# lyeemax/IS-VINS

Measured on AMD Instinct MI355X. Metric: sliding-window solves/sec (11 KF, ~300 landmarks), higher is better.
Workload: dtype f64; 1 GPU; 1024 independent synthetic sliding windows per GPU (N=11 KF, Nvo=5, L=300 landmarks, F~1070 reprojection factors each; BASELINE config 4 batch of config-2 windows), full backendOptimization(): NUM_ITERATIONS=10 dogleg iterations + update() + double2vector + MargForward/MargBackward on every window; windows_per_gpu=1024, windows_total=1024, frames=11, landmarks=300, factors_total=1095427

## Files before the change

is-vins_amd/backend.py:

```python
import ctypes as C
import os
import subprocess

import numpy as np

from . import abi

CSRC = os.path.join(os.path.dirname(os.path.abspath(__file__)), "csrc")
LIB_PATH = os.environ.get("ISVINS_LIB") or os.path.join(CSRC, "libisvins_hip.so")
_lib = None

STATUS = {0: "ISV_OK", -1: "ISV_ERR_INVALID_ARG", -2: "ISV_ERR_CAPACITY", -3: "ISV_ERR_NONFINITE",
          -4: "ISV_ERR_DEVICE", -5: "ISV_ERR_UNSUPPORTED"}
EXPORTS = ["isv_abi_version", "isv_backend_create", "isv_backend_destroy", "isv_backend_last_error",
           "isv_backend_optimize", "isv_backend_optimize_batch", "isv_backend_init_factor_graph", "isv_backend_init_factor_graph_batch", "isv_backend_triangulate", "isv_backend_solve_odometry_batch", "isv_backend_linearize",
           "isv_batch_upload", "isv_batch_optimize", "isv_batch_linearize", "isv_batch_download",
           "isv_batch_sync", "isv_batch_last_timing", "isv_batch_last_counts",
           "isv_result_record_doubles", "isv_batch_pack_results",
           "isv_backend_seq_enable", "isv_backend_seq_seed", "isv_backend_seq_frame", "isv_backend_seq_download", "isv_backend_seq_flush", "isv_backend_seq_marg"]


class BackendError(RuntimeError):
    pass


def build(force=False):
    import fcntl
    if not force and subprocess.call(["make", "-s", "-q", "-C", CSRC]) == 0:
        return LIB_PATH
    with open(os.path.join(CSRC, ".build.lock"), "w") as lock:
        fcntl.flock(lock, fcntl.LOCK_EX)
        try:
            if force:
                subprocess.check_call(["make", "-s", "-C", CSRC, "clean"])
            subprocess.check_call(["make", "-s", "-C", CSRC])
        finally:
            fcntl.flock(lock, fcntl.LOCK_UN)
    return LIB_PATH


def load_library():
    global _lib
    if _lib is not None:
        return _lib
    if not os.path.exists(LIB_PATH):
        raise BackendError(f"HIP extension missing: {LIB_PATH} (run __graft_entry__.build())")
    try:
        import torch
    except Exception:
        pass
    lib = C.CDLL(LIB_PATH)
    vp = C.c_void_p
    wpp = C.POINTER(C.POINTER(abi.isv_window_t))
    dp = abi.c_double_p
    lib.isv_abi_version.restype = C.c_int
    lib.isv_backend_create.argtypes = [C.POINTER(abi.isv_config_t), C.POINTER(vp)]
    lib.isv_backend_destroy.argtypes = [vp]; lib.isv_backend_destroy.restype = None
    lib.isv_backend_last_error.argtypes = [vp]; lib.isv_backend_last_error.restype = C.c_char_p
    lib.isv_backend_optimize.argtypes = [vp, C.POINTER(abi.isv_window_t), C.POINTER(abi.isv_summary_t), C.POINTER(abi.isv_marg_result_t)]
    lib.isv_backend_optimize_batch.argtypes = [vp, C.c_int32, wpp, C.POINTER(abi.isv_summary_t), C.POINTER(abi.isv_marg_result_t)]
    lib.isv_backend_init_factor_graph.argtypes = [vp, C.POINTER(abi.isv_window_t), C.POINTER(abi.isv_summary_t), dp]
    lib.isv_backend_init_factor_graph_batch.argtypes = [vp, C.c_int32, wpp, C.POINTER(abi.isv_summary_t), dp]
    lib.isv_backend_triangulate.argtypes = [vp, C.c_int32, wpp]
    lib.isv_backend_solve_odometry_batch.argtypes = [vp, C.c_int32, wpp, C.POINTER(abi.isv_summary_t), C.POINTER(abi.isv_marg_result_t)]
    lib.isv_backend_linearize.argtypes = [vp, C.POINTER(abi.isv_window_t), dp, dp, dp]
    lib.isv_batch_upload.argtypes = [vp, C.c_int32, wpp]
    lib.isv_batch_optimize.argtypes = [vp, C.c_int32]
    lib.isv_batch_linearize.argtypes = [vp, C.c_int32]
    lib.isv_batch_download.argtypes = [vp, C.c_int32, wpp, C.POINTER(abi.isv_summary_t), C.POINTER(abi.isv_marg_result_t)]
    lib.isv_batch_sync.argtypes = [vp]
    lib.isv_batch_last_timing.argtypes = [vp, dp]
    lib.isv_batch_last_counts.argtypes = [vp, C.POINTER(C.c_int64)]
    lib.isv_debug_read.argtypes = [vp, C.c_int32, dp, C.c_int64]
    lib.isv_result_record_doubles.argtypes = [vp]; lib.isv_result_record_doubles.restype = C.c_int64
    lib.isv_batch_pack_results.argtypes = [vp, vp, vp]
    _lib = lib
    return lib


class Backend:
    def __init__(self, n_frames=11, n_vo=5, max_landmarks=1000, max_obs=None, max_batch=1, **kw):
        self.lib = load_library()
        self.cfg = abi.make_config(n_frames, n_vo, max_landmarks=max_landmarks, max_obs=max_obs, max_batch=max_batch, **kw)
        self.h = C.c_void_p()
        rc = self.lib.isv_backend_create(C.byref(self.cfg), C.byref(self.h))
        if rc != 0:
            raise BackendError(f"isv_backend_create failed: {STATUS.get(rc, rc)} (a MI355X and the HIP extension are required; there is no CPU path)")
        self._keep = None

    def close(self):
        if self.h:
            self.lib.isv_backend_destroy(self.h)
            self.h = C.c_void_p()

    def __del__(self):
        try:
            self.close()
        except Exception:
            pass

    def _check(self, rc, what):
        if rc != 0:
            msg = self.lib.isv_backend_last_error(self.h)
            raise BackendError(f"{what}: {STATUS.get(rc, rc)} {msg.decode() if msg else ''}")

    def _ptrs(self, windows):
        cs = [w.c() for w in windows]
        arr = (C.POINTER(abi.isv_window_t) * len(cs))(*[C.pointer(c) for c in cs])
        self._keep = (cs, arr, windows)
        return arr

    def optimize(self, window):
        s, m = self.optimize_batch([window])
        return s[0], m[0]

    def optimize_batch(self, windows):
        n = len(windows)
        sums = (abi.isv_summary_t * n)(); margs = (abi.isv_marg_result_t * n)()
        self._check(self.lib.isv_backend_optimize_batch(self.h, n, self._ptrs(windows), sums, margs), "optimize_batch")
        return list(sums), list(margs)

    def linearize(self, window):
        F, N = window.n_factors, window.N
        ps = np.zeros((max(F, 1), abi.ISV_PROJ_STRIP)); im = np.zeros((N - 1, abi.ISV_IMU_STRIP)); cost = np.zeros(1)
        cw = window.c()
        self._check(self.lib.isv_backend_linearize(self.h, C.byref(cw), abi._p(ps), abi._p(im), abi._p(cost)), "linearize")
# ... 15 lines not shown
        n = len(windows)
        sums = (abi.isv_summary_t * n)(); kld = np.zeros(n)
        self._check(self.lib.isv_backend_init_factor_graph_batch(self.h, n, self._ptrs(windows), sums, abi._p(kld)), "init_factor_graph_batch")
        for w in windows:
            w.n_rollpitch = 0; w.margin_old = 0
        return list(sums), kld

    def triangulate(self, windows):
        self._check(self.lib.isv_backend_triangulate(self.h, len(windows), self._ptrs(windows)), "triangulate")

    def marshal(self, windows):
        return self._ptrs(windows)

    def upload(self, windows, ptrs=None):
        self._check(self.lib.isv_batch_upload(self.h, len(windows), ptrs if ptrs is not None else self._ptrs(windows)), "upload")
        self._n = len(windows)

    def run_optimize(self, sync=True, profile=False):
        self._check(self.lib.isv_batch_optimize(self.h, (1 if sync else 0) | (2 if profile else 0)), "batch_optimize")

    def run_linearize(self, sync=True):
        self._check(self.lib.isv_batch_linearize(self.h, 1 if sync else 0), "batch_linearize")

    def sync(self):
        self._check(self.lib.isv_batch_sync(self.h), "sync")

    def download(self, windows, ptrs=None, as_list=True):
        n = len(windows)
        sums = (abi.isv_summary_t * n)(); margs = (abi.isv_marg_result_t * n)()
        self._check(self.lib.isv_batch_download(self.h, n, ptrs if ptrs is not None else self._ptrs(windows), sums, margs), "download")
        return (list(sums), list(margs)) if as_list else (sums, margs)

    def record_doubles(self):
        return int(self.lib.isv_result_record_doubles(self.h))

    def pack_results(self, device_ptr, stream=None):
        s = C.c_void_p(-1) if stream is None else C.c_void_p(int(stream))
        self._check(self.lib.isv_batch_pack_results(self.h, C.c_void_p(device_ptr), s), "pack_results")

    def last_timing(self):
        out = np.zeros(8)
        self._check(self.lib.isv_batch_last_timing(self.h, abi._p(out)), "last_timing")
        return out

    def last_counts(self):
        out = (C.c_int64 * 8)()
        self._check(self.lib.isv_batch_last_counts(self.h, out), "last_counts")
        return list(out)

    def debug_read(self, what, count):
        out = np.zeros(count)
        self._check(self.lib.isv_debug_read(self.h, what, abi._p(out), count), "debug_read")
        return out
```

is-vins_amd/csrc/isv_backend.hip:

```cpp
#include <hip/hip_runtime.h>
#include <atomic>
#include <chrono>
#include <cstdio>
#include <cstdlib>
#include <cstring>
#include <string>
#include <thread>
#include <sched.h>
#include <vector>
#include <algorithm>
#include "isv_device_types.h"
#include "isv_kernels.h"

#include "isv_batch_buffers.h"

extern "C" int isv_abi_version(void) { return ISV_ABI_VERSION; }

extern "C" const char *isv_backend_last_error(const isv_backend_t *h) { return h ? h->err.c_str() : "null handle"; }

extern "C" void isv_backend_destroy(isv_backend_t *h) {
    if (!h) return;
    (void)hipSetDevice(h->device);
    if (h->graph_exec) (void)hipGraphExecDestroy(h->graph_exec);
    if (h->seq && h->seq_free) h->seq_free(h->seq);
// ... 759 lines not shown
        double *q = o + 16 * N + maxL;
        q[0] = st.x_cost; q[1] = st.initial_cost; q[2] = st.iteration; q[3] = st.termination; q[4] = st.num_successful;
        q[5] = st.radius; q[6] = d.header0[w]; q[7] = Lw;
    }
}

extern "C" int64_t isv_result_record_doubles(const isv_backend_t *h) {
    return h ? 16 * (int64_t)h->cfg.n_frames + h->cfg.max_landmarks + 8 : 0;
}

extern "C" int isv_batch_pack_results(isv_backend_t *h, void *device_dst, void *stream) {
    if (!h || !device_dst || !h->resident) return ISV_ERR_INVALID_ARG;
    ENTER(h);
    DevBatch &d = h->d;
    hipStream_t dst_stream = stream == ISV_STREAM_OF_HANDLE ? h->stream : (hipStream_t)stream;
    if (dst_stream != h->stream) {
        HIPCHK(h, hipEventRecord(h->pk[0], h->stream));
        HIPCHK(h, hipStreamWaitEvent(dst_stream, h->pk[0], 0));
    }
    hipLaunchKernelGGL(k_pack_results, dim3(d.B), dim3(256), 0, dst_stream, d, (double *)device_dst, isv_result_record_doubles(h), h->cfg.max_landmarks);
    HIPCHK(h, hipGetLastError());
    if (dst_stream != h->stream) {
        HIPCHK(h, hipEventRecord(h->pk[1], dst_stream));
        HIPCHK(h, hipStreamWaitEvent(h->stream, h->pk[1], 0));
    }
    return ISV_OK;
}

extern "C" int isv_debug_read(isv_backend_t *h, int32_t what, double *out, int64_t count) {
    if (!h || !out) return ISV_ERR_INVALID_ARG;
    ENTER(h);
    DevBatch &d = h->d; hipStream_t st = h->stream;
    const double *src = nullptr;
    const size_t B = h->capB, NI = B * (size_t)(d.N - 1);
    size_t cap = 0;
    switch (what) {
    case 0: src = d.prior_strip; cap = B * (size_t)d.prior_strip_sz; break;
    case 1: src = d.prior_cost; cap = B * (size_t)d.n_prior_slots; break;
    case 2: src = d.imu_sqrt; cap = NI * 225; break;
    case 3: src = d.fcost; cap = h->capF; break;
    case 4: src = d.imu_cost; cap = NI; break;
    case 5: src = d.pose; cap = B * (size_t)d.N * 7; break;
    case 6: src = d.lam; cap = h->capL; break;
    case 7: src = d.cost; cap = B; break;
    case 22: src = d.strip_ex; cap = h->capF * 12; if (!src) return ISV_ERR_INVALID_ARG; break;
    default: return isv_solver_debug_read(h->d, st, what, out, count, h->capB, h->capL, h->err);
    }
    if (count < 0 || (size_t)count > cap) { h->err = "isv_debug_read: count exceeds the buffer"; return ISV_ERR_INVALID_ARG; }
    if (count == 0) return ISV_OK;
    D2H(out, src, count);
    HIPCHK(h, hipStreamSynchronize(st));
    return ISV_OK;
}
```

is-vins_amd/csrc/isv_kernels.h:

```cpp
#pragma once
#include <hip/hip_runtime.h>
#include <string>
#include <vector>
#include "isv_device_types.h"
#include "isv_solve_plan.h"

__global__ void k_vector2double(DevBatch d);
__global__ void k_imu_prep(DevBatch d, const int32_t *sel);
template <int MODE> __global__ void k_proj_linearize(DevBatch d, const double *pose_src, const double *lam_src, double *fcost_out, int gate);
template <bool JAC> __global__ void k_imu_linearize(DevBatch d, const double *pose_src, const double *sb_src, double *cost_out, int gate);
template <bool JAC> __global__ void k_prior_linearize(DevBatch d, const double *pose_src, const double *sb_src, double *cost_out, int gate);
__global__ void k_cost_reduce(DevBatch d, const double *fcost, const double *imu_cost, const double *prior_cost, double *out, int gate);

struct SolverHost {
    SolveEnv env;
    SolveDevice dev;
    HandlePlan plan;
    UploadShape upload;
    const void *fn[KR_COUNT] = {};
};
const void *isv_solver_kernel(SolverRole r, KernelInst i, bool ex, int nt);
UploadPlan isv_solver_plan_upload(SolverHost &hc, const UploadShape &u);
int isv_solver_alloc(DevBatch &d, SolverHost &hc, size_t B, size_t L, size_t F, std::vector<void *> &allocs, std::string &err);
int isv_solver_enqueue(DevBatch &d, const SolverHost &hc, hipStream_t st, hipStream_t st2, hipEvent_t *fj, int64_t *counts, hipEvent_t *prof_ev, std::string &err);
__global__ void k_triangulate(DevBatch d);
template <bool EX, int LGW> __global__ void k_lin_gram(DevBatch d);
template <int NT, int TPW> __global__ void k_schur_split(DevBatch d, int Gs, int GrMax);
template <int NT, int TPW> __global__ void k_rank1_split(DevBatch d, int GrMax);
__global__ void k_schur_fold(DevBatch d, int GrMax, int NT, int from_partials);
__global__ void k_imu_raw(DevBatch d, const double *pose_src, const double *sb_src, int gate);
__global__ void k_imu_weight(DevBatch d, double *cost_out, int gate);
#define ISV_PROF_FAMILIES 6
enum { ISV_CNT_LINEARIZE, ISV_CNT_SOLVE, ISV_CNT_ELIM, ISV_CNT_WINDOW_ITERS, ISV_CNT_FUSED_VISUAL, ISV_CNT_FUSED_CONTROL, ISV_CNT_SOLVE_ST, ISV_CNT_SPLIT_GROUPS };
struct SolverStage { SolveState *st; double *tc, *tr, *ts; int32_t *ta; isv_marg_result_t *marg; };
hipError_t isv_raise_dynamic_lds(const void *fn, int device, size_t lds);
int isv_upload_build_enqueue(DevBatch &d, const int32_t *optr, const double *obs_raw, int lcap, hipStream_t st);
int isv_solver_download(struct isv_backend *h, int n, isv_summary_t *summary, isv_marg_result_t *marg);
void isv_solver_unpack_window(const SolverStage &stage, int b, isv_summary_t *summary, isv_marg_result_t *marg);
int isv_solver_debug_read(DevBatch &d, hipStream_t st, int what, double *out, int64_t count, size_t capB, size_t capL, std::string &err);
```

is-vins_amd/csrc/isv_marg.hip:

```cpp
#include <hip/hip_runtime.h>
#include "isv_kernels.h"
#include "isv_device_math.h"
#include "isv_proj_factor.h"
#include "isv_prior_factor.h"

#define MT 64
#ifdef ISV_STAMP
#define MSTAMP(k) do { if (t == 0) { unsigned long long now_ = wall_clock64(); d.dbg[(size_t)w * 64 + 32 + (k)] += (double)(now_ - t_last); t_last = now_; } } while (0)
#else
#define MSTAMP(k) do {} while (0)
#endif
#define SYNC() __syncthreads()
template <bool WV> DEV void tsync() {
    if constexpr (WV) {
        __builtin_amdgcn_fence(__ATOMIC_RELEASE, "workgroup");
        __builtin_amdgcn_wave_barrier();
        __builtin_amdgcn_fence(__ATOMIC_ACQUIRE, "workgroup");
    } else __syncthreads();
}

DEV double jr_rsqrt(double x) { double r = __builtin_amdgcn_rsq(x); const double h = 0.5 * x; r = r * fma(-(h * r), r, 1.5); r = r * fma(-(h * r), r, 1.5); return r; }
DEV double jr_rcp(double x) { double r = __builtin_amdgcn_rcp(x); r = r * fma(-x, r, 2.0); r = r * fma(-x, r, 2.0); return r; }
DEV void jr_params(double app, double aqq, double apq, bool rot, double &c, double &sn) {
    const double theta = ((aqq - app) * 0.5) * jr_rcp(apq);
    const double th2 = fma(theta, theta, 1.0);
    const double tv = (theta >= 0 ? 1.0 : -1.0) * jr_rcp(fma(th2, jr_rsqrt(th2), fabs(theta)));
    const double cc = jr_rsqrt(fma(tv, tv, 1.0));
    c = rot ? cc : 1.0; sn = rot ? tv * cc : 0.0;
}
DEV void jr_block(double ca, double sa, double cb, double sb, double b00, double b01, double b10, double b11,
                  double &o00, double &o01, double &o10, double &o11) {
    const double c00 = fma(cb, b00, -(sb * b01)), c01 = fma(sb, b00, cb * b01);
    const double c10 = fma(cb, b10, -(sb * b11)), c11 = fma(sb, b10, cb * b11);
    o00 = fma(ca, c00, -(sa * c10)); o01 = fma(ca, c01, -(sa * c11));
    o10 = fma(sa, c00, ca * c10); o11 = fma(sa, c01, ca * c11);
}
DEV void jr_vec(double c, double sn, double vp, double vq, double &op, double &oq) { op = fma(c, vp, -(sn * vq)); oq = fma(sn, vp, c * vq); }

template <int TS = MT, bool WV = false>
DEV void w_mm(const double *A, const double *B, double *C, int m, int k, int n, int t) {
    for (int e = t; e < m * n; e += TS) { const int i = e / n, j = e % n; double s = 0; for (int p = 0; p < k; p++) s += A[i * k + p] * B[p * n + j]; C[e] = s; }
    tsync<WV>();
}
template <int TS = MT, bool WV = false>
DEV void w_mm_tn(const double *A, const double *B, double *C, int m, int k, int n, int t) {
    for (int e = t; e < m * n; e += TS) { const int i = e / n, j = e % n; double s = 0; for (int p = 0; p < k; p++) s += A[p * m + i] * B[p * n + j]; C[e] = s; }
    tsync<WV>();
}
template <int TS = MT, bool WV = false>
DEV void w_mm_nt(const double *A, const double *B, double *C, int m, int k, int n, int t) {
    for (int e = t; e < m * n; e += TS) { const int i = e / n, j = e % n; double s = 0; for (int p = 0; p < k; p++) s += A[i * k + p] * B[j * k + p]; C[e] = s; }
    tsync<WV>();
}
template <int TS = MT, bool WV = false>
DEV void w_inv(const double *A, int n, double *Inv, double *W, int *piv, int t) {
    const int n2 = 2 * n;
    for (int e = t; e < n * n2; e += TS) { const int i = e / n2, j = e % n2; W[e] = (j < n) ? A[i * n + j] : ((j - n) == i ? 1.0 : 0.0); }
// ... 408 lines not shown
        SYNC();
        int rank = 6;
        if (t == 0) {
            double Aq[36]; for (int k = 0; k < 36; k++) Aq[k] = Lp[k];
            double pv[6], maxp = 0; rank = 0;
            for (int k = 0; k < 6; k++) pv[k] = 0;
            for (int k = 0; k < 6; k++) {
                int pi = k, pj = k; double best = 0;
                for (int i = k; i < 6; i++) for (int j = k; j < 6; j++) if (fabs(Aq[i * 6 + j]) > best) { best = fabs(Aq[i * 6 + j]); pi = i; pj = j; }
                pv[k] = best; if (best > maxp) maxp = best;
                if (best == 0) break;
                for (int j = 0; j < 6; j++) { const double tmp2 = Aq[k * 6 + j]; Aq[k * 6 + j] = Aq[pi * 6 + j]; Aq[pi * 6 + j] = tmp2; }
                for (int i = 0; i < 6; i++) { const double tmp2 = Aq[i * 6 + k]; Aq[i * 6 + k] = Aq[i * 6 + pj]; Aq[i * 6 + pj] = tmp2; }
                for (int i = k + 1; i < 6; i++) { const double f = Aq[i * 6 + k] / Aq[k * 6 + k]; for (int j = k; j < 6; j++) Aq[i * 6 + j] -= f * Aq[k * 6 + j]; }
            }
            for (int k = 0; k < 6; k++) if (pv[k] > 1e-16 * maxp) rank++;
            piv[1] = rank;
        }
        SYNC();
        rank = piv[1];
        if (rank == 6) {
            w_inv(Lp, 6, cov, Wk + 600, piv, t);
            w_mm(sJ, cov, T, 6, 6, 6, t);
            w_mm_nt(T, sJ, covi, 6, 6, 6, t);
        } else {
            for (int e = t; e < 36; e += MT) JU[e] = Lp[e];
            SYNC();
            w_jacobi(JU, 6, wv, Vv, nullptr, t);
            if (t < 6) keep[t] = wv[t] > d.alpha_cut;
            SYNC();
            w_project_cov(sJ, 6, 6, Vv, wv, keep, JU, covi, t);
        }
        w_inv(covi, 6, X, Wk + 600, piv, t);
        double kld = 0;
        if (rank == 6) {
            double *phi = Wk + 448, *pc = Wk + 512;
            w_mm_tn(sJ, X, T, 6, 6, 6, t);
            w_mm(T, sJ, phi, 6, 6, 6, t);
            w_mm(phi, cov, pc, 6, 6, 6, t);
            const double dphi = w_det(phi, 6, Wk + 900, piv, t), dcov = w_det(cov, 6, Wk + 900, piv, t);
            double a = 0; for (int k = 0; k < 6; k++) a += pc[k * 6 + k];
            kld = 0.5 * (a - log(dphi) - log(dcov) - 6);
        }
        w_chol_upper(X, 6, JU, Wk + 800, t);
        for (int e = t; e < 36; e += MT) fp.sqrt_info[e] = JU[e];
        if (t == 0) { out.forward_kld = kld; out.n_marg_landmarks = n0; out.valid = 1; }
        SYNC();
    }
    MSTAMP(4);
}
template __global__ void k_marg_fwd<64>(DevBatch);
template __global__ void k_marg_fwd<256>(DevBatch);

template <int NC>
DEV void jacobi4(double *sA, double *sV, int t) {
    constexpr int n = NC, m = n + (n & 1), half = m / 2, NI = half * half, NN = n * n;
    static_assert(NI <= 128 && half <= 32, "one item per lane of two wavefronts");
    __shared__ double red[8], sink[2], rc[2][32], rs[2][32];
    __shared__ int rp[2][32], rq[2][32];
    for (int e = t; e < NN; e += 256) sV[e] = (e / n == e % n) ? 1.0 : 0.0;
    __syncthreads();
    const bool is_block = t < 128;
    const int e = is_block ? t : t - 128;
    const bool valid = e < NI;
    const int i0 = valid ? e / half : 0, i1 = valid ? e % half : 0;
    auto params = [&](int r, int buf) {
        if (t < half) {
            const int k = t;
            int a = r + k, b = r + m - 1 - k;
            a = a >= m - 1 ? a - (m - 1) : a;
            b = b >= m - 1 ? b - (m - 1) : b;
            a = k == 0 ? m - 1 : a; b = k == 0 ? r : b;
            const int p = a < b ? a : b, q0 = a < b ? b : a, q = q0 < n ? q0 : p;
            const double apq = sA[p * n + q], aqq = sA[q * n + q], app = sA[p * n + p];
            double c, sn;
            jr_params(app, aqq, apq, p != q && apq != 0.0, c, sn);
            rp[buf][k] = p; rq[buf][k] = q; rc[buf][k] = c; rs[buf][k] = sn;
        }
    };
    bool polish = false;
    for (int sweep = 0; sweep < 30; sweep++) {
        double off = 0, dg = 0;
        for (int x = t; x < NN; x += 256) { const int i = x / n, j = x % n; const double v = sA[x]; if (j > i) off += v * v; else if (i == j) dg += v * v; }
        for (int o = 32; o > 0; o >>= 1) { off += __shfl_xor(off, o); dg += __shfl_xor(dg, o); }
        if ((t & 63) == 0) { red[(t >> 6) * 2] = off; red[(t >> 6) * 2 + 1] = dg; }
        params(0, 0);
        __syncthreads();
        off = red[0] + red[2] + red[4] + red[6]; dg = red[1] + red[3] + red[5] + red[7];
        if (off <= 1e-60 || off <= 1e-32 * dg || polish) break;
        if (off <= 1e-28 * dg) polish = true;
        for (int r = 0; r < m - 1; r++) {
            const int buf = r & 1;
            if (is_block) {
                const int p1 = rp[buf][i0], q1 = rq[buf][i0], p2 = rp[buf][i1], q2 = rq[buf][i1];
                const double ca = rc[buf][i0], sa = rs[buf][i0], cb = rc[buf][i1], sb = rs[buf][i1];
                double *const a00 = valid ? sA + p1 * n + p2 : sink, *const a01 = valid ? sA + p1 * n + q2 : sink;
                double *const a10 = valid ? sA + q1 * n + p2 : sink, *const a11 = valid ? sA + q1 * n + q2 : sink;
                const double b00 = *a00, b01 = *a01, b10 = *a10, b11 = *a11;
                double o00, o01, o10, o11;
                jr_block(ca, sa, cb, sb, b00, b01, b10, b11, o00, o01, o10, o11);
                *a00 = o00; *a01 = o01; *a10 = o10; *a11 = o11;
            } else {
                const int p = rp[buf][i0], q = rq[buf][i0];
                const double c = rc[buf][i0], sn = rs[buf][i0];
                const int k0 = 2 * i1, k1 = (2 * i1 + 1 < n) ? 2 * i1 + 1 : k0;
                double *const v0p = valid ? sV + k0 * n + p : sink + 1, *const v0q = valid ? sV + k0 * n + q : sink + 1;
                double *const v1p = valid ? sV + k1 * n + p : sink + 1, *const v1q = valid ? sV + k1 * n + q : sink + 1;
                const double a0 = *v0p, b0 = *v0q, a1 = *v1p, b1 = *v1q;
                double r0p, r0q, r1p, r1q;
                jr_vec(c, sn, a0, b0, r0p, r0q); jr_vec(c, sn, a1, b1, r1p, r1q);
                *v0p = r0p; *v0q = r0q; *v1p = r1p; *v1q = r1q;
            }
            __syncthreads();
            if (r + 1 < m - 1) { params(r + 1, buf ^ 1); __syncthreads(); }
        }
    }
}
template <int NC>
__global__ __launch_bounds__(256) void k_marg_jacobi(DevBatch d) {
    constexpr int n = NC, NN = n * n;
    __shared__ double sA[NN + 1], sV[NN + 1];
    const int w = blockIdx.x, t = threadIdx.x;
    if (!d.margin_old[w] || ISV_SEQ_IDLE(d, w)) return;
#ifdef ISV_STAMP
    unsigned long long t_last = wall_clock64();
#endif
    double *const ws = d.marg_ws + (size_t)w * ISV_MARG_WS;
    for (int e = t; e < NN; e += 256) sA[e] = ws[e];
    jacobi4<NC>(sA, sV, t);
    for (int x = t; x < NN; x += 256) ws[896 + x] = sV[x];
    if (t < n) ws[1344 + t] = sA[t * n + t];
#ifdef ISV_STAMP
    if (t == 0) d.dbg[(size_t)w * 64 + 32 + 6] += (double)(wall_clock64() - t_last);
#endif
}
template __global__ void k_marg_jacobi<21>(DevBatch);

enum { IRJ_RIT = 1, IRJ_S = 2, IRJ_B1 = 4, IRJ_T = 8, IRJ_B2 = 16, IRJ_ALL = 31 };
DEV void imu_raw_jac(const DevBatch &d, size_t f, const double *pi, const double *si, double *M1, int pieces) {
    const double *rec = d.imu_in + f * ISV_IMU_IN;
    const double *pj = pi + 7, *sj = si + 9;
    Quat Qi = q_from_pose(pi), Qj = q_from_pose(pj), Qii = q_inv(Qi);
    const double dt = rec[IMU_DT];
    double dbg[3], tt[3], u[3], o1[3], o2[3], RiT[9], S1[9], S2[9], B1[9], B2[9], L[9], Rr[9], T[9];
    Quat dq = Quat{rec[IMU_DQ + 3], rec[IMU_DQ], rec[IMU_DQ + 1], rec[IMU_DQ + 2]};
    Quat cdq = dq;
    if (pieces & (IRJ_B1 | IRJ_B2)) {
        for (int k = 0; k < 3; k++) dbg[k] = si[6 + k] - rec[IMU_LBG + k];
        m3v(rec + IMU_DQ_DBG, dbg, tt);
        cdq = q_mul(dq, q_delta(tt));
    }
    if (pieces & IRJ_RIT) q_to_R(Qii, RiT);
    if (pieces & IRJ_S) {
        for (int k = 0; k < 3; k++) u[k] = 0.5 * d.G[k] * dt * dt + pj[k] - pi[k] - si[k] * dt;
        q_rot(Qii, u, o1);
        for (int k = 0; k < 3; k++) u[k] = d.G[k] * dt + sj[k] - si[k];
        q_rot(Qii, u, o2);
        skew3(o1, S1); skew3(o2, S2);
    }
    if (pieces & IRJ_B1) {
        Quat aq = q_mul(q_inv(Qj), Qi);
        qleft33(aq, L); qright33(cdq, Rr); m3_mul(L, Rr, B1);
        const double av[3] = {aq.x, aq.y, aq.z}, bv[3] = {cdq.x, cdq.y, cdq.z};
        for (int r = 0; r < 3; r++) for (int c = 0; c < 3; c++) B1[r * 3 + c] += av[r] * (-bv[c]);
    }
    if (pieces & IRJ_T) {
        qleft33(q_mul(q_mul(q_inv(Qj), Qi), dq), L);
        m3_mul(L, rec + IMU_DQ_DBG, T);
    }
    if (pieces & IRJ_B2) qleft33(q_mul(q_mul(q_inv(cdq), Qii), Qj), B2);
    for (int a = 0; a < 3; a++) for (int b = 0; b < 3; b++) {
        const int ab = a * 3 + b;
        if (pieces & IRJ_RIT) {
            M1[(0 + a) * 30 + 0 + b] = -RiT[ab]; M1[(0 + a) * 30 + 6 + b] = -RiT[ab] * dt; M1[(6 + a) * 30 + 6 + b] = -RiT[ab];
            M1[(0 + a) * 30 + 15 + b] = RiT[ab]; M1[(6 + a) * 30 + 21 + b] = RiT[ab];
        }
        if (pieces & IRJ_S) { M1[(0 + a) * 30 + 3 + b] = S1[ab]; M1[(6 + a) * 30 + 3 + b] = S2[ab]; }
        if (pieces & IRJ_B1) M1[(3 + a) * 30 + 3 + b] = -B1[ab];
        if (pieces & IRJ_T) M1[(3 + a) * 30 + 12 + b] = -T[ab];
        if (pieces & IRJ_B2) M1[(3 + a) * 30 + 18 + b] = B2[ab];
    }
}
DEV void imu_raw_copies(const DevBatch &d, size_t f, double *M1, int ab) {
    const double *rec = d.imu_in + f * ISV_IMU_IN;
    const int a = ab / 3, b = ab % 3;
    M1[(0 + a) * 30 + 9 + b] = -rec[IMU_DP_DBA + ab]; M1[(0 + a) * 30 + 12 + b] = -rec[IMU_DP_DBG + ab];
    M1[(6 + a) * 30 + 9 + b] = -rec[IMU_DV_DBA + ab]; M1[(6 + a) * 30 + 12 + b] = -rec[IMU_DV_DBG + ab];
    M1[(9 + a) * 30 + 9 + b] = (a == b) ? -1.0 : 0.0; M1[(12 + a) * 30 + 12 + b] = (a == b) ? -1.0 : 0.0;
    M1[(9 + a) * 30 + 24 + b] = (a == b) ? 1.0 : 0.0; M1[(12 + a) * 30 + 27 + b] = (a == b) ? 1.0 : 0.0;
// ... 74 lines not shown
    } else if (t == 0) {
        const size_t f = (size_t)w * (N - 1) + (v - 1);
        imu_raw_jac(d, f, pose + 7 * (v - 1), sb + 9 * (v - 1), M1, IRJ_ALL);
        for (int ab = 0; ab < 9; ab++) imu_raw_copies(d, f, M1, ab);
    }
    SYNC();
    {
        const double *S = d.imu_sqrt + ((size_t)w * (N - 1) + (v - 1)) * 225;
        for (int e = t; e < 450; e += NTH) { const int a = e / 30, c = e % 30; double s = 0; for (int k = 0; k < 15; k++) s += S[a * 15 + k] * M1[k * 30 + c]; M2[e] = s; }
        SYNC();
        for (int e = t; e < 900; e += NTH) {
            const int a = e / 30, b = e % 30;
            const int ga = (a < 15) ? 15 + a : a - 15, gb = (b < 15) ? 15 + b : b - 15;
            double s = 0; for (int k = 0; k < 15; k++) s += M2[k * 30 + a] * M2[k * 30 + b];
            Lam[ga * 30 + gb] += s;
        }
        SYNC();
    }
    double *Lp = M1;
    {
        double *A99 = Wk, *Ainv = Wk + 100;
        for (int e = t; e < 81; e += NTH) A99[e] = Lam[(21 + e / 9) * 30 + 21 + e % 9];
        SYNC();
        if constexpr (PART == 3) { if (wid == 0) w_inv<64, true>(A99, 9, Ainv, Wk + 200, piv, lane); SYNC(); }
        else w_inv(A99, 9, Ainv, Wk + 200, piv, t);
        for (int e = t; e < 441; e += NTH) {
            const int a = e / 21, b = e % 21; double s = Lam[a * 30 + b];
#pragma unroll SCHUR_UNROLL
            for (int p = 0; p < 9; p++) { double tt = 0; for (int q = 0; q < 9; q++) tt += Ainv[p * 9 + q] * Lam[b * 30 + 21 + q]; s -= Lam[a * 30 + 21 + p] * tt; }
            Lp[e] = s;
        }
        SYNC();
    }
    if constexpr (PART == 3) {
        for (int e = t; e < 441; e += NTH) Jr[e] = recovered_jac_entry(e / 21, e % 21, sJ, wv);
    } else {
        for (int e = t; e < 441; e += MT) Jr[e] = 0.0;
        SYNC();
        if (t == 0) {
            double BmBy[9];
            recovered_jac(pose, sb, v, rp, vb, gp, sJ, BmBy);
            for (int a = 0; a < 6; a++) for (int b = 0; b < 6; b++) { Jr[a * 21 + 15 + b] += sJ[a * 6 + b]; Jr[a * 21 + b] += sJ[36 + a * 6 + b]; }
            for (int a = 0; a < 9; a++) Jr[(6 + a) * 21 + 6 + a] += 1.0;
            for (int a = 0; a < 2; a++) for (int b = 0; b < 3; b++) Jr[(15 + a) * 21 + 18 + b] += BmBy[a * 3 + b];
            for (int a = 0; a < 3; a++) Jr[(17 + a) * 21 + 15 + a] += 1.0;
            for (int b = 0; b < 3; b++) Jr[20 * 21 + 18 + b] += BmBy[6 + b];
        }
    }
    SYNC();
    if constexpr (PART == 0) for (int e = t; e < 441; e += MT) { ws[e] = Lp[e]; ws[448 + e] = Jr[e]; }
    MSTAMP(5);
    if constexpr (PART == 3) {
        for (int e = t; e < 441; e += NTH) M2[e] = Lp[e];
        jacobi4<21>(M2, Vv, t);
        if (t < 21) { const double ev = M2[t * 21 + t]; wv[t] = ev; keep[t] = ev > d.alpha_cut; }
        SYNC();
        MSTAMP(6);
    }
    if constexpr (PART == 2) {
        for (int e = t; e < 441; e += MT) M2[e] = Lp[e];
        SYNC();
        w_jacobi(M2, 21, wv, Vv, nullptr, t);
        if (t < 21) keep[t] = wv[t] > d.alpha_cut;
        SYNC();
        MSTAMP(6);
    }
    }
    if constexpr (PART == 1) {
        for (int e = t; e < 441; e += MT) { Jr[e] = ws[448 + e]; Vv[e] = ws[896 + e]; }
        if (t < 21) { const double ev = ws[1344 + t]; wv[t] = ev; keep[t] = ev > d.alpha_cut; }
        SYNC();
    }
    if constexpr (PART != 0) {
    {
        double *Sg = Wk, *Xi = Wk + 100, *Xall = M1;
        for (int e = t; e < 441; e += NTH) Xall[e] = 0.0;
        SYNC();
#define RECOVER_ON(WV, TT, R0, NR, DST, JUp, Sgp, Xip, Wp, Lp_, PV)                                                     \
        do {                                                                                                            \
            w_project_cov<MT, WV>(Jr + (R0) * 21, (NR), 21, Vv, wv, keep, (JUp), (Sgp), (TT));                          \
            w_inv<MT, WV>((Sgp), (NR), (Xip), (Wp), (PV), (TT));                                                        \
            for (int e = (TT); e < (NR) * (NR); e += MT) Xall[((R0) + e / (NR)) * 21 + (R0) + e % (NR)] = (Xip)[e];    \
            tsync<WV>();                                                                                                \
            if ((DST) != nullptr) {                                                                                     \
                w_chol_upper<MT, WV>((Xip), (NR), (Sgp), (Lp_), (TT));                                                  \
                for (int e = (TT); e < (NR) * (NR); e += MT) (DST)[e] = (Sgp)[e];                                       \
                tsync<WV>();                                                                                            \
            }                                                                                                           \
        } while (0)
#define RECOVER(R0, NR, DST) RECOVER_ON(false, t, R0, NR, DST, JU, Sg, Xi, Wk + 300, Wk + 200, piv)
        double *const no_dst = nullptr;
        if constexpr (PART == 3) {
            if (wid == 0) RECOVER_ON(true, lane, 6, 9, vb.sqrt_info, JU + 6 * 21, Sg, Xi, Wk + 300, Wk + 200, piv);
            else if (wid == 1) RECOVER_ON(true, lane, 0, 6, rp.sqrt_info, JU, M2, M2 + 36, M2 + 72, M2 + 144, piv + 1);
            else if (wid == 2) {
                RECOVER_ON(true, lane, 15, 2, gp.sqrt_info, JU + 15 * 21, M2 + 200, M2 + 210, M2 + 220, M2 + 240, piv + 2);
                RECOVER_ON(true, lane, 17, 3, no_dst, JU + 17 * 21, M2 + 200, M2 + 210, M2 + 220, M2 + 240, piv + 2);
                RECOVER_ON(true, lane, 20, 1, no_dst, JU + 20 * 21, M2 + 200, M2 + 210, M2 + 220, M2 + 240, piv + 2);
            }
            SYNC();
        } else {
            RECOVER(0, 6, rp.sqrt_info);
            RECOVER(6, 9, vb.sqrt_info);
            RECOVER(15, 2, gp.sqrt_info);
            RECOVER(17, 3, no_dst);
            RECOVER(20, 1, no_dst);
        }
// ... 201 lines not shown
```

Baseline: 211,600 windows/s.

## Pipeline Jacobi rotation parameters with double-buffered matrix to halve barriers per round

Restructures the 4-wavefront parallel Jacobi eigensolver used in marginalization. One wavefront now computes the next round's rotation parameters speculatively, gathering 2x2 blocks via DPP quad broadcasts from precomputed offset tables, while the others apply the current rotations into a ping-pong buffer. This removes the second barrier per round and the serialized params step. Eigenvector updates are regrouped so that lanes own rows. It adds a second 21x21 shared buffer, heavier index math, and a debug hook for testing the kernel in isolation.

```diff
diff --git a/is-vins_amd/backend.py b/is-vins_amd/backend.py
--- a/is-vins_amd/backend.py
+++ b/is-vins_amd/backend.py
@@ -72,6 +72,8 @@
     lib.isv_batch_last_timing.argtypes = [vp, dp]
     lib.isv_batch_last_counts.argtypes = [vp, C.POINTER(C.c_int64)]
     lib.isv_debug_read.argtypes = [vp, C.c_int32, dp, C.c_int64]
+    if hasattr(lib, "isv_debug_jacobi"):
+        lib.isv_debug_jacobi.argtypes = [vp, C.c_int32, dp, C.c_int64, dp, dp]
     lib.isv_result_record_doubles.argtypes = [vp]; lib.isv_result_record_doubles.restype = C.c_int64
     lib.isv_batch_pack_results.argtypes = [vp, vp, vp]
     _lib = lib
@@ -193,3 +195,9 @@
         out = np.zeros(count)
         self._check(self.lib.isv_debug_read(self.h, what, abi._p(out), count), "debug_read")
         return out
+
+    def debug_jacobi(self, mats, waves=4):
+        a = np.ascontiguousarray(mats, dtype=np.float64).reshape(-1, 21, 21)
+        V = np.zeros_like(a); w = np.zeros((a.shape[0], 21))
+        self._check(self.lib.isv_debug_jacobi(self.h, waves, abi._p(a), a.shape[0], abi._p(V), abi._p(w)), "debug_jacobi")
+        return V, w
diff --git a/is-vins_amd/csrc/isv_backend.hip b/is-vins_amd/csrc/isv_backend.hip
--- a/is-vins_amd/csrc/isv_backend.hip
+++ b/is-vins_amd/csrc/isv_backend.hip
@@ -835,3 +835,9 @@
     HIPCHK(h, hipStreamSynchronize(st));
     return ISV_OK;
 }
+
+extern "C" int isv_debug_jacobi(isv_backend_t *h, int32_t waves, const double *A, int64_t count, double *V, double *w) {
+    if (!h) return ISV_ERR_INVALID_ARG;
+    ENTER(h);
+    return isv_marg_debug_jacobi(h->d, h->stream, waves, A, count, V, w, h->capB, h->err);
+}
diff --git a/is-vins_amd/csrc/isv_jacobi_schedule.h b/is-vins_amd/csrc/isv_jacobi_schedule.h
--- /dev/null
+++ b/is-vins_amd/csrc/isv_jacobi_schedule.h
@@ -0,0 +1,48 @@
+#pragma once
+#if defined(__HIPCC__)
+#define JS_HD __host__ __device__ inline
+#else
+#define JS_HD inline
+#endif
+
+struct JsPair { int p, q; };
+
+JS_HD int js_players(int n) { return n + (n & 1); }
+JS_HD int js_wrap(int x, int M) { return x >= M ? x - M : x; }
+
+JS_HD JsPair js_pair(int n, int r, int k) {
+    const int M = js_players(n) - 1;
+    int a = js_wrap(r + k, M), b = js_wrap(r + M - k, M);
+    if (k == 0) { a = M; b = r; }
+    const int lo = a < b ? a : b, hi = a < b ? b : a;
+    JsPair pr; pr.p = lo; pr.q = hi < n ? hi : lo;
+    return pr;
+}
+JS_HD JsPair js_pair_moving(int n, int r, int k) {
+    const int M = js_players(n) - 1;
+    const int a = js_wrap(r + k, M), b = js_wrap(r + M - k, M);
+    JsPair pr; pr.p = a < b ? a : b; pr.q = a < b ? b : a;
+    return pr;
+}
+JS_HD int js_pair_of(int n, int r, int i) {
+    const int m = js_players(n), M = m - 1, half = m / 2;
+    if (i == M) return 0;
+    const int d = js_wrap(i + M - r, M);
+    return d == 0 ? 0 : (d < half ? d : M - d);
+}
+JS_HD void js_entry_block(int n, int r, int i, int j, int &ka, int &kb, int &slot) {
+    ka = js_pair_of(n, r, i); kb = js_pair_of(n, r, j);
+    slot = 2 * (i == js_pair(n, r, ka).q) + (j == js_pair(n, r, kb).q);
+}
+JS_HD bool js_priority(int n, int r, int k, int s, int &i, int &j) {
+    const int M = js_players(n) - 1;
+    const JsPair nx = js_pair(n, js_wrap(r + 1, M), k);
+    i = s == 1 ? nx.q : nx.p; j = s == 0 ? nx.p : nx.q;
+    return s == 0 || (s < 3 && nx.p != nx.q);
+}
+
+JS_HD int js_index(int n, int r, int off) { const int M = js_players(n) - 1; return off < 0 ? M : js_wrap(r + off, M); }
+JS_HD int js_member_offset(int n, int k, int mu) { const int M = js_players(n) - 1; return k == 0 ? (mu == 0 ? -1 : 0) : (mu == 0 ? k : M - k); }
+JS_HD int js_prev_offset(int n, int off) { const int M = js_players(n) - 1; return off < 0 ? -1 : js_wrap(off + 1, M); }
+JS_HD int js_pair_of_offset(int n, int off) { const int m = js_players(n), M = m - 1, half = m / 2; return off <= 0 ? 0 : (off < half ? off : M - off); }
+JS_HD int js_partner_offset(int n, int off) { const int M = js_players(n) - 1; return off < 0 ? 0 : (off == 0 ? -1 : M - off); }
diff --git a/is-vins_amd/csrc/isv_kernels.h b/is-vins_amd/csrc/isv_kernels.h
--- a/is-vins_amd/csrc/isv_kernels.h
+++ b/is-vins_amd/csrc/isv_kernels.h
@@ -38,3 +38,4 @@
 int isv_solver_download(struct isv_backend *h, int n, isv_summary_t *summary, isv_marg_result_t *marg);
 void isv_solver_unpack_window(const SolverStage &stage, int b, isv_summary_t *summary, isv_marg_result_t *marg);
 int isv_solver_debug_read(DevBatch &d, hipStream_t st, int what, double *out, int64_t count, size_t capB, size_t capL, std::string &err);
+int isv_marg_debug_jacobi(DevBatch &d, hipStream_t st, int waves, const double *A, int64_t count, double *V, double *wv, size_t capB, std::string &err);
diff --git a/is-vins_amd/csrc/isv_marg.hip b/is-vins_amd/csrc/isv_marg.hip
--- a/is-vins_amd/csrc/isv_marg.hip
+++ b/is-vins_amd/csrc/isv_marg.hip
@@ -3,6 +3,7 @@
 #include "isv_device_math.h"
 #include "isv_proj_factor.h"
 #include "isv_prior_factor.h"
+#include "isv_jacobi_schedule.h"
 
 #define MT 64
 #ifdef ISV_STAMP
@@ -517,89 +518,184 @@
 template __global__ void k_marg_fwd<64>(DevBatch);
 template __global__ void k_marg_fwd<256>(DevBatch);
 
+#define JAC_LDS_BARRIER() do { __builtin_amdgcn_fence(__ATOMIC_RELEASE, "workgroup", "local"); __builtin_amdgcn_s_barrier(); __builtin_amdgcn_fence(__ATOMIC_ACQUIRE, "workgroup", "local"); } while (0)
+template <int L> DEV double quad_bcast(double x) {
+    constexpr int ctrl = L * 0x55;
+    const int xl = __double2loint(x), xh = __double2hiint(x);
+    return __hiloint2double(__builtin_amdgcn_update_dpp(xh, xh, ctrl, 0xF, 0xF, false), __builtin_amdgcn_update_dpp(xl, xl, ctrl, 0xF, 0xF, false));
+}
+#ifdef ISV_STAMP
+#define JSTAMP(acc) do { const unsigned long long n_ = wall_clock64(); (acc) += n_ - jt_; jt_ = n_; } while (0)
+#else
+#define JSTAMP(acc) do {} while (0)
+#endif
 template <int NC>
-DEV void jacobi4(double *sA, double *sV, int t) {
-    constexpr int n = NC, m = n + (n & 1), half = m / 2, NI = half * half, NN = n * n;
-    static_assert(NI <= 128 && half <= 32, "one item per lane of two wavefronts");
+DEV void jacobi4(double *sA, double *sB, double *sV, int t, double *stamp = nullptr) {
+    constexpr int n = NC, m = n + (n & 1), M = m - 1, half = m / 2, NI = half * half, NN = n * n, VG = (half + 3) / 4;
+    static_assert(NI <= 128 && 4 * half <= 64 && VG * n <= 64, "a priority quad per pair on one wavefront, a block per lane on two, VG eigenvector lanes per row on one");
     __shared__ double red[8], sink[2], rc[2][32], rs[2][32];
-    __shared__ int rp[2][32], rq[2][32];
+#ifdef ISV_STAMP
+    unsigned long long jt_ = 0, jb_ = 0, jp_ = 0, js_ = 0;
+#endif
     for (int e = t; e < NN; e += 256) sV[e] = (e / n == e % n) ? 1.0 : 0.0;
-    __syncthreads();
-    const bool is_block = t < 128;
-    const int e = is_block ? t : t - 128;
-    const bool valid = e < NI;
-    const int i0 = valid ? e / half : 0, i1 = valid ? e % half : 0;
-    auto params = [&](int r, int buf) {
-        if (t < half) {
-            const int k = t;
-            int a = r + k, b = r + m - 1 - k;
-            a = a >= m - 1 ? a - (m - 1) : a;
-            b = b >= m - 1 ? b - (m - 1) : b;
-            a = k == 0 ? m - 1 : a; b = k == 0 ? r : b;
-            const int p = a < b ? a : b, q0 = a < b ? b : a, q = q0 < n ? q0 : p;
-            const double apq = sA[p * n + q], aqq = sA[q * n + q], app = sA[p * n + p];
-            double c, sn;
-            jr_params(app, aqq, apq, p != q && apq != 0.0, c, sn);
-            rp[buf][k] = p; rq[buf][k] = q; rc[buf][k] = c; rs[buf][k] = sn;
-        }
+    const int wid = t >> 6, lane = t & 63;
+    const int pr_k = (lane >> 2) < half ? lane >> 2 : 0, pr_s = lane & 3;
+    const bool pr_write = (lane >> 2) < half && pr_s == 0, pr_real = !((n & 1) && pr_k == 0);
+    const int pr_d0 = js_prev_offset(n, js_member_offset(n, pr_k, 0)), pr_d1 = js_prev_offset(n, js_member_offset(n, pr_k, 1));
+    const int pr_di = (pr_s & 1) ? pr_d1 : pr_d0, pr_dj = (pr_s == 1 || pr_s == 2) ? pr_d1 : pr_d0;
+    const int pr_dip = js_partner_offset(n, pr_di), pr_djp = js_partner_offset(n, pr_dj);
+    const int pr_ka = js_pair_of_offset(n, pr_di), pr_kb = js_pair_of_offset(n, pr_dj);
+    const int e = wid == 3 ? lane : t - 64;
+    const bool valid = wid == 3 ? e < VG * n : (wid != 0 && e < NI);
+    const int i0 = valid ? (wid == 3 ? e / n : e / half) : 0, i1 = valid ? (wid == 3 ? e % n : e % half) : 0;
+    static_assert(NN * 8 < 65536, "offsets in 16 bits");
+    __shared__ unsigned ptab[2][2][64];
+    auto row_word = [&](int r) -> unsigned {
+        const int i = js_index(n, r, pr_di), ip = js_index(n, r, pr_dip);
+        const int r0 = i < ip ? i : ip, r1m = i < ip ? ip : i, r1 = r1m < n ? r1m : r0;
+        return (unsigned)(r0 * n * 8) | (unsigned)(r1 * n * 8) << 16 | (i == r1 ? 1u : 0u);
     };
+    auto col_word = [&](int r) -> unsigned {
+        const int j = js_index(n, r, pr_dj), jp = js_index(n, r, pr_djp);
+        const int c0 = j < jp ? j : jp, c1m = j < jp ? jp : j, c1 = c1m < n ? c1m : c0;
+        return (unsigned)(c0 * 8) | (unsigned)(c1 * 8) << 16 | (j == c1 ? 1u : 0u) | (js_index(n, r, pr_d0) > js_index(n, r, pr_d1) ? 2u : 0u);
+    };
+    unsigned er = row_word(0), ec = col_word(0);
+    if (wid == 1) ptab[1][0][lane] = row_word(js_wrap(1, M));
+    if (wid == 2) ptab[1][1][lane] = col_word(js_wrap(1, M));
+    double *cur = sA, *nxt = sB;
+    int buf = 0;
     bool polish = false;
     for (int sweep = 0; sweep < 30; sweep++) {
+        if (sweep == 0) JAC_LDS_BARRIER();
         double off = 0, dg = 0;
-        for (int x = t; x < NN; x += 256) { const int i = x / n, j = x % n; const double v = sA[x]; if (j > i) off += v * v; else if (i == j) dg += v * v; }
+        for (int y = t; y < NN; y += 256) { const int i = y / n, j = y % n; const double v = cur[y]; if (j > i) off += v * v; else if (i == j) dg += v * v; }
         for (int o = 32; o > 0; o >>= 1) { off += __shfl_xor(off, o); dg += __shfl_xor(dg, o); }
         if ((t & 63) == 0) { red[(t >> 6) * 2] = off; red[(t >> 6) * 2 + 1] = dg; }
-        params(0, 0);
-        __syncthreads();
+        if (sweep == 0 && t < half) {
+            const JsPair pq = js_pair(n, 0, t);
+            const double apq = cur[pq.p * n + pq.q], aqq = cur[pq.q * n + pq.q], app = cur[pq.p * n + pq.p];
+            double c, sn;
+            jr_params(app, aqq, apq, pq.p != pq.q && apq != 0.0, c, sn);
+            rc[0][t] = c; rs[0][t] = sn;
+        }
+        JAC_LDS_BARRIER();
         off = red[0] + red[2] + red[4] + red[6]; dg = red[1] + red[3] + red[5] + red[7];
         if (off <= 1e-60 || off <= 1e-32 * dg || polish) break;
         if (off <= 1e-28 * dg) polish = true;
-        for (int r = 0; r < m - 1; r++) {
-            const int buf = r & 1;
-            if (is_block) {
-                const int p1 = rp[buf][i0], q1 = rq[buf][i0], p2 = rp[buf][i1], q2 = rq[buf][i1];
-                const double ca = rc[buf][i0], sa = rs[buf][i0], cb = rc[buf][i1], sb = rs[buf][i1];
-                double *const a00 = valid ? sA + p1 * n + p2 : sink, *const a01 = valid ? sA + p1 * n + q2 : sink;
-                double *const a10 = valid ? sA + q1 * n + p2 : sink, *const a11 = valid ? sA + q1 * n + q2 : sink;
-                const double b00 = *a00, b01 = *a01, b10 = *a10, b11 = *a11;
+#ifdef ISV_STAMP
+        jt_ = wall_clock64(); js_++;
+#endif
+        for (int r = 0; r < M; r++) {
+            if (wid == 0) {
+                const char *const base = (const char *)cur;
+                const unsigned ro0 = er & 0xfff8u, ro1 = (er >> 16) & 0xfff8u, co0 = ec & 0xfff8u, co1 = (ec >> 16) & 0xfff8u;
+                const double ca = rc[buf][pr_ka], sa = rs[buf][pr_ka], cb = rc[buf][pr_kb], sb = rs[buf][pr_kb];
+                const double b00 = *(const double *)(base + ro0 + co0), b01 = *(const double *)(base + ro0 + co1);
+                const double b10 = *(const double *)(base + ro1 + co0), b11 = *(const double *)(base + ro1 + co1);
+                const unsigned ern = ptab[buf ^ 1][0][lane], ecn = ptab[buf ^ 1][1][lane];
                 double o00, o01, o10, o11;
                 jr_block(ca, sa, cb, sb, b00, b01, b10, b11, o00, o01, o10, o11);
-                *a00 = o00; *a01 = o01; *a10 = o10; *a11 = o11;
+                const double v0 = (er & 1) ? ((ec & 1) ? o11 : o10) : ((ec & 1) ? o01 : o00);
+                const double v1 = quad_bcast<1>(v0), v2 = quad_bcast<2>(v0), v3 = quad_bcast<3>(v0);
+                const bool ba = (ec & 2) != 0;
+                const double app = ba ? v1 : v0, aqq = ba ? v0 : v1, apq = ba ? v3 : v2;
+                JSTAMP(jb_);
+                double c, sn;
+                jr_params(app, aqq, apq, pr_real && apq != 0.0, c, sn);
+                if (pr_write) { rc[buf ^ 1][pr_k] = c; rs[buf ^ 1][pr_k] = sn; }
+                er = ern; ec = ecn;
+            } else if (wid < 3) {
+                const JsPair pa = js_pair(n, r, i0), pb = js_pair(n, r, i1);
+                const double ca = rc[buf][i0], sa = rs[buf][i0], cb = rc[buf][i1], sb = rs[buf][i1];
+                const int x00 = pa.p * n + pb.p, x01 = pa.p * n + pb.q, x10 = pa.q * n + pb.p, x11 = pa.q * n + pb.q;
+                const double b00 = cur[x00], b01 = cur[x01], b10 = cur[x10], b11 = cur[x11];
+                double o00, o01, o10, o11;
+                jr_block(ca, sa, cb, sb, b00, b01, b10, b11, o00, o01, o10, o11);
+                *(valid ? nxt + x00 : sink) = o00; *(valid ? nxt + x01 : sink) = o01; *(valid ? nxt + x10 : sink) = o10; *(valid ? nxt + x11 : sink) = o11;
+                const int r2 = js_wrap(js_wrap(r + 1, M) + 1, M);
+                if (wid == 1) ptab[buf][0][lane] = row_word(r2); else ptab[buf][1][lane] = col_word(r2);
             } else {
-                const int p = rp[buf][i0], q = rq[buf][i0];
-                const double c = rc[buf][i0], sn = rs[buf][i0];
-                const int k0 = 2 * i1, k1 = (2 * i1 + 1 < n) ? 2 * i1 + 1 : k0;
-                double *const v0p = valid ? sV + k0 * n + p : sink + 1, *const v0q = valid ? sV + k0 * n + q : sink + 1;
-                double *const v1p = valid ? sV + k1 * n + p : sink + 1, *const v1q = valid ? sV + k1 * n + q : sink + 1;
-                const double a0 = *v0p, b0 = *v0q, a1 = *v1p, b1 = *v1q;
-                double r0p, r0q, r1p, r1q;
-                jr_vec(c, sn, a0, b0, r0p, r0q); jr_vec(c, sn, a1, b1, r1p, r1q);
-                *v0p = r0p; *v0q = r0q; *v1p = r1p; *v1q = r1q;
+                double *const row = sV + i1 * n;
+#pragma unroll
+                for (int g = 0; g < 4; g++) {
+                    const int k = 4 * i0 + g < half ? 4 * i0 + g : half - 1;
+                    const bool on = valid && 4 * i0 + g < half;
+                    const JsPair pq = g == 0 ? js_pair(n, r, k) : js_pair_moving(n, r, k);
+                    const double c = rc[buf][k], sn = rs[buf][k];
+                    double *const vp = on ? row + pq.p : sink + 1, *const vq = on ? row + pq.q : sink + 1;
+                    const double a0 = *vp, b0 = *vq;
+                    double r0p, r0q;
+                    jr_vec(c, sn, a0, b0, r0p, r0q);
+                    *vp = r0p; *vq = r0q;
+                }
             }
-            __syncthreads();
-            if (r + 1 < m - 1) { params(r + 1, buf ^ 1); __syncthreads(); }
-        }
-    }
+            JAC_LDS_BARRIER();
+            if (wid == 0) JSTAMP(jp_);
+            double *const sw = cur; cur = nxt; nxt = sw;
+            buf ^= 1;
+        }
+    }
+    if (cur != sA) {
+        for (int x = t; x < NN; x += 256) sA[x] = cur[x];
+        JAC_LDS_BARRIER();
+    }
+#ifdef ISV_STAMP
+    if (t == 0 && stamp) { stamp[0] += (double)jb_; stamp[1] += (double)jp_; stamp[2] += (double)js_; }
+#endif
+}
+template <int NC>
+DEV void marg_jacobi_ws(double *ws, int t) {
+    constexpr int n = NC, NN = n * n;
+    __shared__ double sA[NN + 1], sB[NN + 1], sV[NN + 1];
+    for (int e = t; e < NN; e += 256) sA[e] = ws[e];
+    jacobi4<NC>(sA, sB, sV, t);
+    for (int x = t; x < NN; x += 256) ws[896 + x] = sV[x];
+    if (t < n) ws[1344 + t] = sA[t * n + t];
 }
 template <int NC>
 __global__ __launch_bounds__(256) void k_marg_jacobi(DevBatch d) {
-    constexpr int n = NC, NN = n * n;
-    __shared__ double sA[NN + 1], sV[NN + 1];
     const int w = blockIdx.x, t = threadIdx.x;
     if (!d.margin_old[w] || ISV_SEQ_IDLE(d, w)) return;
 #ifdef ISV_STAMP
     unsigned long long t_last = wall_clock64();
 #endif
-    double *const ws = d.marg_ws + (size_t)w * ISV_MARG_WS;
-    for (int e = t; e < NN; e += 256) sA[e] = ws[e];
-    jacobi4<NC>(sA, sV, t);
-    for (int x = t; x < NN; x += 256) ws[896 + x] = sV[x];
-    if (t < n) ws[1344 + t] = sA[t * n + t];
+    marg_jacobi_ws<NC>(d.marg_ws + (size_t)w * ISV_MARG_WS, t);
 #ifdef ISV_STAMP
     if (t == 0) d.dbg[(size_t)w * 64 + 32 + 6] += (double)(wall_clock64() - t_last);
 #endif
 }
 template __global__ void k_marg_jacobi<21>(DevBatch);
+
+template <int WAVES>
+__global__ __launch_bounds__(64 * WAVES) void k_jacobi_hook(double *ws_all) {
+    double *const ws = ws_all + (size_t)blockIdx.x * ISV_MARG_WS;
+    const int t = threadIdx.x;
+    if constexpr (WAVES == 4) marg_jacobi_ws<21>(ws, t);
+    else {
+        __shared__ double hA[442], hV[442], hw[32];
+        for (int e = t; e < 441; e += MT) hA[e] = ws[e];
+        SYNC();
+        w_jacobi_pipe<21>(hA, hw, hV, t);
+        for (int e = t; e < 441; e += MT) ws[896 + e] = hV[e];
+        if (t < 21) ws[1344 + t] = hw[t];
+    }
+}
+int isv_marg_debug_jacobi(DevBatch &d, hipStream_t st, int waves, const double *A, int64_t count, double *V, double *wv, size_t capB, std::string &err) {
+    if ((waves != 1 && waves != 4) || !A || !V || !wv || count < 0 || (size_t)count > capB) { err = "isv_debug_jacobi: waves is 1 or 4, count at most max_batch"; return ISV_ERR_INVALID_ARG; }
+    if (count == 0) return ISV_OK;
+#define JCHK(call) do { hipError_t e_ = (call); if (e_ != hipSuccess) { err = std::string(#call) + ": " + hipGetErrorString(e_); return ISV_ERR_DEVICE; } } while (0)
+    const size_t pitch = sizeof(double) * ISV_MARG_WS;
+    JCHK(hipMemcpy2DAsync(d.marg_ws, pitch, A, sizeof(double) * 441, sizeof(double) * 441, (size_t)count, hipMemcpyHostToDevice, st));
+    if (waves == 4) hipLaunchKernelGGL(k_jacobi_hook<4>, dim3((unsigned)count), dim3(256), 0, st, d.marg_ws);
+    else hipLaunchKernelGGL(k_jacobi_hook<1>, dim3((unsigned)count), dim3(64), 0, st, d.marg_ws);
+    JCHK(hipGetLastError());
+    JCHK(hipMemcpy2DAsync(V, sizeof(double) * 441, d.marg_ws + 896, pitch, sizeof(double) * 441, (size_t)count, hipMemcpyDeviceToHost, st));
+    JCHK(hipMemcpy2DAsync(wv, sizeof(double) * 21, d.marg_ws + 1344, pitch, sizeof(double) * 21, (size_t)count, hipMemcpyDeviceToHost, st));
+    JCHK(hipStreamSynchronize(st));
+#undef JCHK
+    return ISV_OK;
+}
 
 enum { IRJ_RIT = 1, IRJ_S = 2, IRJ_B1 = 4, IRJ_T = 8, IRJ_B2 = 16, IRJ_ALL = 31 };
 DEV void imu_raw_jac(const DevBatch &d, size_t f, const double *pi, const double *si, double *M1, int pieces) {
@@ -780,7 +876,11 @@
     MSTAMP(5);
     if constexpr (PART == 3) {
         for (int e = t; e < 441; e += NTH) M2[e] = Lp[e];
-        jacobi4<21>(M2, Vv, t);
+#ifdef ISV_STAMP
+        jacobi4<21>(M2, M1, Vv, t, d.dbg + (size_t)w * 64 + 45);
+#else
+        jacobi4<21>(M2, M1, Vv, t);
+#endif
         if (t < 21) { const double ev = M2[t * 21 + t]; wv[t] = ev; keep[t] = ev > d.alpha_cut; }
         SYNC();
         MSTAMP(6);
```

Result: no change. 210,200 windows/s (-0.6%).
